# fgnt/pb_chime5

Measured on AMD Instinct MI355X. Metric: utterance-seconds enhanced/sec/GPU (24ch, 20 EM iters), higher is better.
Workload: dtype f64

## Files before the change

### pb_chime5_amd/csrc/gss_api.hip

```cpp
#include <cmath>
#include <cstdarg>
#include <cstdlib>
#include <cstring>
#include <mutex>

#include "gss_internal.h"

#define GSS_ENTER(ctx)                                   \
    if (!(ctx)) return GSS_ERR_INVALID;                  \
    GSS_HIP_CHECK((ctx), hipSetDevice((ctx)->device))
#define GSS_ENTER_VARIANTS(ctx) \
    GSS_ENTER(ctx);             \
    GSS_TRY(variant_refresh(ctx))
static int variant_refresh(gss_ctx *ctx);

#define GSS_STATUS_REF_CHANNEL 0
#define GSS_STATUS_WPE_ZERO_PIVOTS 2

static std::mutex g_error_lock;

int gss_fail(gss_ctx *ctx, int code, const char *fmt, ...) {
    char buf[1024];
    va_list ap;
    va_start(ap, fmt);
    vsnprintf(buf, sizeof(buf), fmt, ap);
    va_end(ap);
    if (ctx) {
        std::lock_guard<std::mutex> guard(g_error_lock);
        ctx->error = buf;
    }
    return code;
}

static thread_local std::string g_create_error;

namespace {
const char *const kVariantKeys[] = {
    "corr_ts", "corr_nw", "corr_blocked", "corr_p_tiles", "chol_diag_unfolded", "apply_ph",
    "apply_generic", "prof_detail", "corr_stg8", "corr_ksplit", "apply_gglobal", "wpe_halves",
    "em_wgs", "estep_wpb", "estep_lds", "mstep_prefetch_d", "mstep_tiled", "mstep_plan_min_d",
    "mstep_chunked", "mstep_slots", "force_eigh", "em_unfused", "em_l3_mb", "em_l3_fit_mb",
    "em_streams", "mstep_maxseg", "em4_cold_eigh", "mstep_generic",
    "wpe_online_mem"};
struct VariantTable {
    std::mutex lock;
    std::string text;
    bool parsed = false;
    std::map<std::string, int> values;
};
VariantTable &variant_table() {
    static VariantTable t;
    return t;
}
}

static int variant_refresh(gss_ctx *ctx) {
    const char *env = getenv("GSS_VARIANT");
    VariantTable &t = variant_table();
    std::lock_guard<std::mutex> guard(t.lock);
    if (t.parsed && t.text == (env ? env : "")) return GSS_OK;
    t.text = env ? env : "";
    t.parsed = true;
// ... 2677 lines not shown
```

### pb_chime5_amd/csrc/wpe.hip

```cpp
#include <algorithm>
#include <cmath>
#include <cstdlib>

#include "gss_internal.h"
#include <type_traits>
#include "dense_wave.h"

typedef double v4d __attribute__((ext_vector_type(4)));

namespace {

constexpr int POW_FRAMES = 256;
__global__ __launch_bounds__(POW_FRAMES) void wpe_power_kernel(const cplx *__restrict__ X,
                                                               int64_t T, int D, int psd_context,
                                                               double *__restrict__ raw,
                                                               double *__restrict__ w) {
    extern __shared__ __attribute__((aligned(16))) char smem[];
    double *ps = reinterpret_cast<double *>(smem);
    __shared__ double red[POW_FRAMES / 64];
    const int f = blockIdx.x, tid = threadIdx.x;
    const cplx *Xf = X + (int64_t)f * T * D;
    double *wout = w + (int64_t)f * T;
    double *wf = psd_context > 0 ? raw + (int64_t)f * T : wout;
    const int DP = D + 1;
// ... 75 lines not shown
                wout[t] = p;
                mx = fmax(mx, p);
            }
        }
    }
    mx = wave_max(mx);
    if ((tid & 63) == 0) red[tid >> 6] = mx;
    __syncthreads();
    mx = fmax(fmax(red[0], red[1]), fmax(red[2], red[3]));
    const double eps = 1e-10 * mx;
    for (int64_t t = tid; t < T; t += POW_FRAMES) wout[t] = 1.0 / fmax(wout[t], eps);
}

#ifndef GSS_CORR_KT
#define GSS_CORR_KT 64
#endif
constexpr int CORR_KT = GSS_CORR_KT;
constexpr int CORR_FINE_MAX_SUBTILES = 48;

struct CorrTile {
    int row_off, col_off, is_p, mask;
};

template <int TS, int MASK, int KSTEPS = CORR_KT / 4>
__device__ __forceinline__ void corr_chunk(const cplx *S, const double *wS, int D,
                                           const CorrTile &tl, v4d (&t1)[TS][TS],
                                           v4d (&t2)[TS][TS], v4d (&t3)[TS][TS]) {
    const int lane = threadIdx.x & 63;
    const int li = lane & 15, lk = lane >> 4;
    auto need = [](int a, int b) { return ((MASK >> (a * TS + b)) & 1) != 0; };
    auto need_row = [&](int a) {
        bool r = false;
        for (int b = 0; b < TS; ++b) r = r || need(a, b);
        return r;
    };
    auto need_col = [&](int b) {
        bool r = false;
        for (int a = 0; a < TS; ++a) r = r || need(a, b);
        return r;
    };
    const int ksteps = KSTEPS;
    cplx a_cur[TS], b_cur[TS], a_nxt[TS], b_nxt[TS];
    double w_cur, w_nxt = 0.0;
    {
        const cplx *base = S + lk * D + li;
        w_cur = wS[lk];
#pragma unroll
        for (int m = 0; m < TS; ++m) {
            a_cur[m] = base[tl.row_off + 16 * m];
            b_cur[m] = base[tl.col_off + 16 * m];
        }
    }
    constexpr int KU = TS == 1 || KSTEPS < 16 ? 4 : 16;
#pragma unroll KU
    for (int ks = 0; ks < ksteps; ++ks) {
        if (ks + 1 < ksteps) {
            const int kf = 4 * (ks + 1) + lk;
            const cplx *base = S + kf * D + li;
            w_nxt = wS[kf];
#pragma unroll
            for (int m = 0; m < TS; ++m) {
                a_nxt[m] = need_row(m) ? base[tl.row_off + 16 * m] : c_make(0.0, 0.0);
                b_nxt[m] = need_col(m) ? base[tl.col_off + 16 * m] : c_make(0.0, 0.0);
            }
        }
        double ar[TS], ai[TS], as[TS], br[TS], bi[TS], bd[TS];
#pragma unroll
        for (int m = 0; m < TS; ++m) {
            ar[m] = a_cur[m].x * w_cur;
            ai[m] = a_cur[m].y * w_cur;
            as[m] = ar[m] + ai[m];
            br[m] = b_cur[m].x;
            bi[m] = b_cur[m].y;
            bd[m] = b_cur[m].x - b_cur[m].y;
        }
#pragma unroll
        for (int a = 0; a < TS; ++a)
#pragma unroll
            for (int b = 0; b < TS; ++b) {
                if (!need(a, b)) continue;
                t1[a][b] = __builtin_amdgcn_mfma_f64_16x16x4f64(ar[a], br[b], t1[a][b], 0, 0, 0);
                t2[a][b] = __builtin_amdgcn_mfma_f64_16x16x4f64(ai[a], bi[b], t2[a][b], 0, 0, 0);
                t3[a][b] = __builtin_amdgcn_mfma_f64_16x16x4f64(as[a], bd[b], t3[a][b], 0, 0, 0);
            }
#pragma unroll
        for (int m = 0; m < TS; ++m) {
            a_cur[m] = a_nxt[m];
            b_cur[m] = b_nxt[m];
        }
        w_cur = w_nxt;
    }
}

template <int TS, int MASK, bool RAW = false>
__device__ __forceinline__ void corr_store(const CorrTile &tl, int f, int n, int c, int D,
                                           const v4d (&t1)[TS][TS], const v4d (&t2)[TS][TS],
                                           const v4d (&t3)[TS][TS], cplx *__restrict__ R,
                                           cplx *__restrict__ P) {
    const int lane = threadIdx.x & 63;
    const int li = lane & 15, lk = lane >> 4;
    auto need = [](int a, int b) { return ((MASK >> (a * TS + b)) & 1) != 0; };
    cplx *Rf = R + (int64_t)f * n * n;
    cplx *Pf = P + (int64_t)f * n * D;
#pragma unroll
    for (int a = 0; a < TS; ++a)
#pragma unroll
        for (int b = 0; b < TS; ++b)
#pragma unroll
            for (int reg = 0; reg < 4; ++reg) {
                if (!need(a, b)) continue;
                const int r = tl.row_off + 16 * a + lk + 4 * reg;
                const int cc = tl.col_off + 16 * b + li;
                const cplx v = RAW ? c_make(t1[a][b][reg], t3[a][b][reg])
                                   : c_make(t1[a][b][reg] + t2[a][b][reg],
                                            (t3[a][b][reg] - t1[a][b][reg]) + t2[a][b][reg]);
                if (r >= n) continue;
                if (tl.is_p == 1) {
                    const int d = cc - c * D;
                    if (d >= 0 && d < D) Pf[r * D + d] = v;
                } else {
                    if (cc < n) Rf[r * n + cc] = v;
                    if (tl.is_p == 2) {
                        const int d = cc - c * D;
                        if (d >= 0 && d < D) Pf[r * D + d] = v;
                    }
                }
            }
}

template <int TS>
__device__ __forceinline__ void corr_zero(v4d (&t1)[TS][TS], v4d (&t2)[TS][TS], v4d (&t3)[TS][TS]) {
#pragma unroll
    for (int a = 0; a < TS; ++a)
#pragma unroll
        for (int b = 0; b < TS; ++b) {
// ... 57 lines not shown
template <int TS, int NW, int STG1 = 8>
__global__ __launch_bounds__(64 * NW, (NW == 1 && STG1 < 8) ? 4 : 1) void wpe_corr_kernel(
    const cplx *__restrict__ Y, const double *__restrict__ w, int F, int64_t T, int D, int n,
    int c, int padf, const CorrTile *__restrict__ tiles, int ntiles, cplx *__restrict__ R,
    cplx *__restrict__ P) {
    extern __shared__ __attribute__((aligned(16))) char smem[];
    const int frames_lds = CORR_KT + c + padf;
    cplx *S = reinterpret_cast<cplx *>(smem);
    double *wS = reinterpret_cast<double *>(S + frames_lds * D);

    int f, grp;
    if (!xcd_group_map((ntiles + NW - 1) / NW, F, f, grp)) return;
    const int wave = __builtin_amdgcn_readfirstlane(threadIdx.x >> 6);
    const int tile_id = grp * NW + wave;
    const bool active = tile_id < ntiles;
    const CorrTile tl = tiles[active ? tile_id : 0];
    const cplx *Yf = Y + (int64_t)f * T * D;
    const double *wf = w + (int64_t)f * T;
    constexpr int FULL = (1 << (TS * TS)) - 1;
    const int mask = __builtin_amdgcn_readfirstlane(active ? tl.mask : 1);
#define CORR_CASE(M) \
    case M: corr_tile_body<TS, M, NW, STG1>(Yf, wf, T, D, n, c, frames_lds, S, wS, tl, active, f, R, P); break
    if (TS == 2) {
        switch (mask) {
            CORR_CASE(1);
            CORR_CASE(3);
            CORR_CASE(5);
            CORR_CASE(11);
            default:
                corr_tile_body<TS, FULL, NW, STG1>(Yf, wf, T, D, n, c, frames_lds, S, wS, tl, active, f, R, P);
        }
    } else {
        corr_tile_body<TS, FULL, NW, STG1>(Yf, wf, T, D, n, c, frames_lds, S, wS, tl, active, f, R, P);
    }
#undef CORR_CASE
}

template <int KS, int STG>
__global__ __launch_bounds__(64 * KS, 4) void wpe_corr_ksplit_kernel(
    const cplx *__restrict__ Y, const double *__restrict__ w, int F, int64_t T, int D, int n,
    int c, int padf, const CorrTile *__restrict__ tiles, int ntiles, cplx *__restrict__ R,
    cplx *__restrict__ P) {
    extern __shared__ __attribute__((aligned(16))) char smem[];
    const int frames_lds = CORR_KT + c + padf;
    const int total = frames_lds * D;
    const size_t wbytes = sizeof(cplx) * (size_t)total + sizeof(double) * CORR_KT;
    int f, tile_id;
// ... 251 lines not shown
        }
    };

    int item = __builtin_amdgcn_readfirstlane(ring[0]);
    if (item < 0) return;
    int b = 0;
    issue(item >> 12, 0, 0);
    __syncthreads();
    for (int k = 0; item >= 0; ++k) {
        const int next = __builtin_amdgcn_readfirstlane(ring[(k + 1) % 3]);
        int fetched = -1;
        if (threadIdx.x == 0 && next >= 0) fetched = corr_fetch(counters, F, xcd, live, cq);
        const int f = item >> 12, grp = item & 4095;
        const int tile_id = grp * NW + wave;
        const bool active = tile_id < ntiles;
        const CorrTile tl = tiles[active ? tile_id : 0];
        const int mask = __builtin_amdgcn_readfirstlane(active ? tl.mask : 1);
        int *ring_slot = &ring[(k + 2) % 3];
#define CORR_CASE(M)                                                                              \
    case M:                                                                                       \
        corr_item_dma<M, NW, BLOCKED>(T, D, n, c, win, S0, w0, tl, active, f, next < 0 ? -1 : next >> 12, \
                                 b, issue, ring_slot, fetched, R, P);                             \
        break
        switch (mask) {
            CORR_CASE(1);
            CORR_CASE(3);
            CORR_CASE(5);
            CORR_CASE(11);
            default:
                corr_item_dma<15, NW, BLOCKED>(T, D, n, c, win, S0, w0, tl, active, f,
                                          next < 0 ? -1 : next >> 12, b, issue, ring_slot, fetched,
                                          R, P);
        }
#undef CORR_CASE
        item = next;
#ifdef GSS_CORR_TRACE
        if (threadIdx.x == 0 && blockIdx.x < 8192) {
            g_corr_trace[blockIdx.x * 6 + 3] = wall_clock64();
            g_corr_trace[blockIdx.x * 6 + 4] = clock64();
            g_corr_trace[blockIdx.x * 6 + 5] = k + 1;
        }
#endif
    }
}

#ifndef GSS_UPD_PREFETCH
#define GSS_UPD_PREFETCH 1
#endif
constexpr int CH_NB = 48;
constexpr int UD_LD = CH_NB + 1;

constexpr size_t DIAG_LDS = sizeof(cplx) * 2 * UD_LD + sizeof(double) * CH_NB;

__device__ inline void chol_diag_block(cplx *A, int n, int j0, cplx *Ud, double *dinv,
                                       int32_t *zero_pivots) {
    const int tid = threadIdx.x, tx = tid & 15, ty = tid >> 4;
    const int nb = min(CH_NB, n - j0);
// ... 439 lines not shown
                    }
                    nxim[it] = -xim[it];
#pragma unroll
                    for (int reg = 0; reg < 4; ++reg) {
                        const int rl = 16 * it + lk + 4 * reg, col = c0 + 16 * b + li;
                        if (rl < nb && col < D)
                            Z[(int64_t)(j0 + rl) * D + col] = c_make(xre[it][reg], xim[it][reg]);
                    }
                }
            }
            __syncthreads();
        }
    }
}

__global__ __launch_bounds__(256, 3) void chol_backsolve_kernel(const cplx *__restrict__ R,
                                                             cplx *__restrict__ P, int n, int D) {
    __shared__ cplx S[CH_NB * BS_LD];
    __shared__ cplx OP[BS_OPS];
    const int f = blockIdx.x;
    chol_backsolve_body(R + (int64_t)f * n * n, P + (int64_t)f * n * D, n, D, S, OP);
}

template <int TA, int NB, int NWV = 4, int WRAPS = 4, bool TAIL = true>
__global__ __launch_bounds__(64 * NWV) void wpe_apply_kernel(const cplx *__restrict__ Y,
                                                        const cplx *__restrict__ G, int F,
                                                        int64_t T, int D, int n, int c,
                                                        cplx *__restrict__ X) {
    constexpr int WAVE_FRAMES = 16 * TA, WG_FRAMES = NWV * WAVE_FRAMES;
    extern __shared__ __attribute__((aligned(16))) char smem[];
    cplx *S = reinterpret_cast<cplx *>(smem);
    const int DP = D | 1;
    int f, chunk;
    if (!xcd_group_map((int)((T + WG_FRAMES - 1) / WG_FRAMES), F, f, chunk)) return;
    const int64_t t0 = (int64_t)chunk * WG_FRAMES;
    const cplx *Yf = Y + (int64_t)f * T * D;
    const cplx *Gf = G + (int64_t)f * n * D;
    const int frames_lds = WG_FRAMES + c + 2;
    const int64_t fr0 = t0 - c;
    constexpr int PRE = 14, NT = 64 * NWV;
    const int total = frames_lds * D;
    for (int base = 0; base < total; base += NT * PRE) {
        cplx v[PRE];
#pragma unroll
        for (int j = 0; j < PRE; ++j) {
            const int idx = base + (int)threadIdx.x + NT * j;
            const int64_t fr = fr0 + idx / D;
            v[j] = c_make(0.0, 0.0);
            if (idx < total && fr >= 0 && fr < T) v[j] = Yf[fr0 * D + idx];
        }
#pragma unroll
        for (int j = 0; j < PRE; ++j) {
            const int idx = base + (int)threadIdx.x + NT * j;
            const int fl = idx / D, d = idx - fl * D;
            if (idx < total) S[fl * DP + d] = v[j];
        }
    }
    __syncthreads();
    const int wave = threadIdx.x >> 6, lane = threadIdx.x & 63;
    const int li = lane & 15, lk = lane >> 4;
    const int wf0 = wave * WAVE_FRAMES;
    if (t0 + wf0 >= T) return;
    v4d acc_re[TA][NB], acc_im[TA][NB], acc_t2[TA][NB];
#pragma unroll
    for (int a = 0; a < TA; ++a)
#pragma unroll
        for (int b = 0; b < NB; ++b) {
            acc_re[a][b] = (v4d){0.0, 0.0, 0.0, 0.0};
            acc_im[a][b] = (v4d){0.0, 0.0, 0.0, 0.0};
            acc_t2[a][b] = (v4d){0.0, 0.0, 0.0, 0.0};
        }
    const int ksteps = (n + 3) / 4;
    const int lds_last = frames_lds * DP - 1;
    int goff[NB], goff_max[NB];
#pragma unroll
    for (int b = 0; b < NB; ++b) {
        const int col = min(16 * b + li, D - 1);
        goff[b] = min(lk, n - 1) * D + col;
        goff_max[b] = (n - 1) * D + col;
    }
    auto load_g = [&](int, cplx (&g)[NB]) {
#pragma unroll
        for (int b = 0; b < NB; ++b) {
            g[b] = Gf[goff[b]];
            goff[b] = min(goff[b] + 4 * D, goff_max[b]);
        }
    };
    int rm = lk % D, lin = (lk / D) * DP + rm;
    int ubase[TA];
#pragma unroll
    for (int a = 0; a < TA; ++a) ubase[a] = (wf0 + 16 * a + li) * DP;
    auto load_u = [&](cplx (&u)[TA]) {
#pragma unroll
        for (int a = 0; a < TA; ++a) u[a] = S[min(ubase[a] + lin, lds_last)];
        rm += 4;
        lin += 4;
#pragma unroll
        for (int w = 0; w < WRAPS; ++w) {
            const bool wrap = rm >= D;
            rm -= wrap ? D : 0;
            lin += wrap ? DP - D : 0;
        }
    };
    auto step = [&](int ks, const cplx (&g)[NB], const cplx (&u)[TA]) {
        const bool ok = !TAIL || 4 * ks + lk < n;
        double ur[TA], ui[TA], gr[NB], gi[NB];
#pragma unroll
        for (int a = 0; a < TA; ++a) {
            ur[a] = ok ? u[a].x : 0.0;
            ui[a] = ok ? u[a].y : 0.0;
        }
#pragma unroll
        for (int b = 0; b < NB; ++b) {
            gr[b] = g[b].x;
            gi[b] = g[b].y;
        }
        double us[TA], gd[NB];
#pragma unroll
        for (int a = 0; a < TA; ++a) us[a] = ur[a] + ui[a];
#pragma unroll
        for (int b = 0; b < NB; ++b) gd[b] = gr[b] - gi[b];
#pragma unroll
        for (int a = 0; a < TA; ++a)
#pragma unroll
            for (int b = 0; b < NB; ++b) {
                acc_re[a][b] = __builtin_amdgcn_mfma_f64_16x16x4f64(ur[a], gr[b], acc_re[a][b], 0, 0, 0);
                acc_t2[a][b] = __builtin_amdgcn_mfma_f64_16x16x4f64(ui[a], gi[b], acc_t2[a][b], 0, 0, 0);
                acc_im[a][b] = __builtin_amdgcn_mfma_f64_16x16x4f64(us[a], gd[b], acc_im[a][b], 0, 0, 0);
            }
    };
    cplx g0[NB], g1[NB], u0[TA], u1[TA];
    load_g(0, g0);
    load_u(u0);
    for (int ks = 0; ks < ksteps; ks += 2) {
        load_g(ks + 1, g1);
        load_u(u1);
        __builtin_amdgcn_sched_barrier(0);
        step(ks, g0, u0);
        __builtin_amdgcn_sched_barrier(0);
        load_g(ks + 2, g0);
        load_u(u0);
        __builtin_amdgcn_sched_barrier(0);
        step(ks + 1, g1, u1);
        __builtin_amdgcn_sched_barrier(0);
    }
#pragma unroll
    for (int a = 0; a < TA; ++a)
#pragma unroll
        for (int b = 0; b < NB; ++b)
#pragma unroll
            for (int reg = 0; reg < 4; ++reg) {
                const int fl = wf0 + 16 * a + lk + 4 * reg;
                const int d = 16 * b + li;
                const int64_t t = t0 + fl;
                if (d < D && t < T) {
                    const cplx y = S[(fl + c) * DP + d];
                    const double pre = acc_re[a][b][reg] + acc_t2[a][b][reg];
                    const double pim = (acc_im[a][b][reg] - acc_re[a][b][reg]) + acc_t2[a][b][reg];
                    X[((int64_t)f * T + t) * D + d] = c_make(y.x - pre, y.y - pim);
                }
            }
}

template <int PH, int NT, bool GLDS = true, int PREW = 14, int PREG = 14>
__global__ __launch_bounds__(256) void wpe_apply_packed_kernel(const cplx *__restrict__ Y,
                                                               const cplx *__restrict__ G, int F,
                                                               int64_t T, int D, int n, int c,
                                                               cplx *__restrict__ X) {
    constexpr int WG_ROWS = 64, WG_FRAMES = PH * WG_ROWS;
    extern __shared__ __attribute__((aligned(16))) char smem[];
    const int DP = D | 1, DG = GLDS ? (D | 1) : D;
    const int frames_lds = WG_FRAMES + c + 2;
    cplx *S = reinterpret_cast<cplx *>(smem);
    cplx *Gl = S + (frames_lds * DP + frames_lds / PH + 1);
    int f, chunk;
    if (!xcd_group_map((int)((T + WG_FRAMES - 1) / WG_FRAMES), F, f, chunk)) return;
    const int64_t t0 = (int64_t)chunk * WG_FRAMES;
    const cplx *Yf = Y + (int64_t)f * T * D;
    const cplx *Gf = G + (int64_t)f * n * D;
    const int64_t fr0 = t0 - c;
    constexpr int NTHR = 256;
    {
        constexpr int PRE = PREW;
        const int total = frames_lds * D;
// ... 195 lines not shown
            const int fl = PH * r + colp[b];
            const int64_t t = t0 + fl;
            if (colv[b] && t < T) {
                const int fw = fl + c;
                const cplx y = S[fw * DP + fw / PH + cold[b]];
                const double pre = acc_re[b][reg] + acc_t2[b][reg];
                const double pim = (acc_im[b][reg] - acc_re[b][reg]) + acc_t2[b][reg];
                X[((int64_t)f * T + t) * D + cold[b]] = c_make(y.x - pre, y.y - pim);
            }
        }
}

__global__ void mfma_selftest_kernel(double *out) {
    const int lane = threadIdx.x;
    const int li = lane & 15, lk = lane >> 4;
    const double a = lk == 0 ? (double)(li + 1) : 0.0;
    const double b = lk == 0 ? 100.0 * (double)(li + 1) : 0.0;
    v4d acc = {0.0, 0.0, 0.0, 0.0};
    acc = __builtin_amdgcn_mfma_f64_16x16x4f64(a, b, acc, 0, 0, 0);
    for (int reg = 0; reg < 4; ++reg) {
        const int row = lk + 4 * reg, col = li;
        out[row * 16 + col] = acc[reg];
    }
}

constexpr int REGROUP_FRAMES = 32;
constexpr int REGROUP_THREADS = 256;

template <bool to_arrays>
__global__ __launch_bounds__(REGROUP_THREADS) void wpe_arrays_regroup_kernel(
    const cplx *__restrict__ src, int64_t T, int A, int C, cplx *__restrict__ dst) {
    __shared__ cplx tile[REGROUP_FRAMES * GSS_MAX_CHANNELS];
    const int D = A * C;
    const int64_t f = blockIdx.y;
    const int64_t t0 = (int64_t)blockIdx.x * REGROUP_FRAMES;
    const int nt = (int)std::min<int64_t>(REGROUP_FRAMES, T - t0);
    const int64_t ftd0 = (f * T + t0) * D;
    const int n_ftd = nt * D;
    if (to_arrays) {
        for (int k = threadIdx.x; k < n_ftd; k += REGROUP_THREADS) tile[k] = src[ftd0 + k];
    } else {
        for (int k = threadIdx.x; k < n_ftd; k += REGROUP_THREADS) {
            const int a = k / (nt * C), r = k - a * nt * C;
            const int t = r / C, c = r - t * C;
            tile[t * D + a * C + c] = src[((f * A + a) * T + t0) * C + r];
        }
// ... 7 lines not shown
        }
    } else {
        for (int k = threadIdx.x; k < n_ftd; k += REGROUP_THREADS) dst[ftd0 + k] = tile[k];
    }
}

}

int wpe_arrays_regroup_run(gss_ctx *ctx, const cplx *src, int F, int64_t T, int A, int C,
                           bool to_arrays, cplx *dst) {
    GSS_REQUIRE(ctx, A * C <= GSS_MAX_CHANNELS, GSS_ERR_UNSUPPORTED, "regroup: D=%d", A * C);
    const dim3 grid((unsigned)((T + REGROUP_FRAMES - 1) / REGROUP_FRAMES), (unsigned)F);
    GSS_PROF(ctx, "wpe_arrays_regroup");
    if (to_arrays)
        hipLaunchKernelGGL(wpe_arrays_regroup_kernel<true>, grid, dim3(REGROUP_THREADS), 0,
                           ctx->stream, src, T, A, C, dst);
    else
        hipLaunchKernelGGL(wpe_arrays_regroup_kernel<false>, grid, dim3(REGROUP_THREADS), 0,
                           ctx->stream, src, T, A, C, dst);
    GSS_LAUNCH_CHECK(ctx, "wpe_arrays_regroup_kernel");
    return GSS_OK;
}

static int corr_tiles(int n, int D, int c, int ct, std::vector<CorrTile> &tiles) {
    const int ts = ct / 16;
    auto mask_of = [&](int r0, int c0, int ncols_limit, bool upper_only) {
        int m = 0;
        for (int a = 0; a < ts; ++a)
            for (int b = 0; b < ts; ++b) {
                const int rr = r0 + 16 * a, cc = c0 + 16 * b;
                bool needed = rr < n && cc < ncols_limit;
                if (upper_only && cc + 15 < rr) needed = false;
                if (needed) m |= 1 << (a * ts + b);
            }
        return m;
    };
    const int last_col = (n - 1) / ct;
    const bool p_folded = ct == 16 && (c * D) / ct == last_col && (c * D + D - 1) / ct == last_col &&
                          !gss_variant_set("corr_p_tiles");
    for (int r0 = 0; r0 < n; r0 += ct)
        for (int c0 = 0; c0 < n; c0 += ct)
            if (c0 + ct > r0) {
                const bool with_p = p_folded && c0 / ct == last_col;
                tiles.push_back({r0, c0, with_p ? 2 : 0,
                                 mask_of(r0, c0, with_p ? std::max(n, c * D + D) : n, true)});
            }
    if (!p_folded)
        for (int r0 = 0; r0 < n; r0 += ct)
            for (int c0 = 0; c0 < D; c0 += ct)
                tiles.push_back({r0, c * D + c0, 1, mask_of(r0, c0, D, false)});
    std::stable_sort(tiles.begin(), tiles.end(), [](const CorrTile &x, const CorrTile &y) {
        return __builtin_popcount(x.mask) > __builtin_popcount(y.mask);
    });
    return (int)tiles.size();
}

static int corr_tiles_pairs(int n, int D, int c, std::vector<CorrTile> &tiles) {
    for (int r0 = 0; r0 < n; r0 += 16)
        for (int c0 = r0; c0 < n; c0 += 32) tiles.push_back({r0, c0, 0, c0 + 16 < n ? 3 : 1});
    for (int r0 = 0; r0 < n; r0 += 32)
        for (int c0 = 0; c0 < D; c0 += 16) tiles.push_back({r0, c * D + c0, 1, r0 + 16 < n ? 5 : 1});
    std::stable_sort(tiles.begin(), tiles.end(), [](const CorrTile &x, const CorrTile &y) {
        return __builtin_popcount(x.mask) > __builtin_popcount(y.mask);
    });
    return (int)tiles.size();
}

static int corr_padf(int D, int ct) { return (ct + D - 1) / D + 1; }

struct WpeWork {
    double *w, *raw;
    cplx *R, *P;
};
static WpeWork wpe_blocks(Workspace &ws, int F, int64_t T, int D, int taps, bool own_w,
                          bool smoothed) {
// ... 51 lines not shown
        if (X != Y)
            GSS_HIP_CHECK(ctx, hipMemcpyAsync(X, Y, sizeof(cplx) * (size_t)F * T * D,
                                              hipMemcpyDeviceToDevice, ctx->stream));
        return GSS_OK;
    }
    GSS_REQUIRE(ctx, X != Y, GSS_ERR_INVALID, "gss_wpe: X must not alias Y");
    GSS_REQUIRE(ctx, !cw || (cw->w && iterations == 1 && part < 0), GSS_ERR_INVALID,
                "wpe: the caller's weights serve one iteration of a whole call");
    Workspace ws(ctx);
    const WpeWork k = wpe_blocks(ws, F, T, D, taps, !cw, psd_context > 0);
    GSS_TRY(ws.status("wpe"));
    double *w_own = k.w, *raw = k.raw;
    const double *w = cw ? cw->w : w_own;
    cplx *R = k.R, *P = k.P;

    std::vector<CorrTile> tiles;
    const int sub16 = (n + 15) / 16;
    int corr_ts = sub16 * (sub16 + 1) / 2 + sub16 * ((D + 15) / 16) <= CORR_FINE_MAX_SUBTILES ? 1 : 2;
    bool corr_pairs = false;
    if (const int e = gss_variant("corr_ts", 0)) {
        corr_ts = e == 1 ? 1 : 2;
        corr_pairs = e == 3;
    }
    const int ntiles = corr_pairs ? corr_tiles_pairs(n, D, c, tiles) : corr_tiles(n, D, c, 16 * corr_ts, tiles);
    constexpr int tm16 = 16, tn16 = 16;
    std::vector<UpdTile> upd;
    std::vector<int> upd_start, upd_count, upd_j0, upd_k, upd_ndiag;
    const bool fold_diag = !gss_variant_set("chol_diag_unfolded");
    {
        const int nblk = (n + CH_NB - 1) / CH_NB;
        for (int J = 0; J < nblk; ++J) {
            upd_start.push_back((int)upd.size());
            const int rs = (J + 1) * CH_NB;
            const bool narrow = J % 2 == 0;
            const int r_end = narrow ? std::min(rs + CH_NB, n) : n;
            const int d_end = std::min(rs + CH_NB, n);
            for (int r0 = rs; r0 < d_end; r0 += tm16)
                for (int c0 = rs; c0 < d_end; c0 += tn16)
                    if (c0 + tn16 > r0) upd.push_back({r0, c0, 0, 0});
            upd_ndiag.push_back(fold_diag ? (int)upd.size() - upd_start.back() : 0);
            for (int r0 = rs; r0 < r_end; r0 += tm16) {
                for (int c0 = rs; c0 < n; c0 += tn16)
                    if (c0 + tn16 > r0 && !(r0 < d_end && c0 < d_end)) upd.push_back({r0, c0, 0, 0});
                for (int cc = 0; cc < D; cc += tn16) upd.push_back({r0, cc, 1, 0});
            }
            upd_count.push_back((int)upd.size() - upd_start.back());
            const bool wide = J % 2 == 1;
            upd_j0.push_back(wide ? (J - 1) * CH_NB : J * CH_NB);
            upd_k.push_back(wide ? 2 * CH_NB : CH_NB);
        }
    }
    GSS_REQUIRE(ctx, ntiles <= 1024 && upd.size() <= 4096, GSS_ERR_UNSUPPORTED,
                "wpe: taps*D=%d too large", n);
    static_assert(sizeof(CorrTile) == sizeof(UpdTile), "tile structs share one buffer");
    if (ctx->wpe_tiles_key[0] != taps || ctx->wpe_tiles_key[1] != delay ||
        ctx->wpe_tiles_key[2] != D || ctx->wpe_tiles_key[3] != corr_ts + (fold_diag ? 0 : 16) + (corr_pairs ? 32 : 0)) {
        GSS_HIP_CHECK(ctx, hipStreamSynchronize(ctx->stream));
        if (!ctx->wpe_tiles)
            GSS_HIP_CHECK(ctx, hipMalloc(&ctx->wpe_tiles, sizeof(CorrTile) * (1024 + 4096 + 1 + 64)));
        if (ctx->debug_pattern >= 0)
            GSS_HIP_CHECK(ctx, hipMemset(ctx->wpe_tiles, ctx->debug_pattern,
                                         sizeof(CorrTile) * (1024 + 4096 + 1 + 64)));
        GSS_HIP_CHECK(ctx, hipMemcpy(ctx->wpe_tiles, tiles.data(), sizeof(CorrTile) * ntiles,
                                     hipMemcpyHostToDevice));
        if (!upd.empty())
            GSS_HIP_CHECK(ctx, hipMemcpy(reinterpret_cast<CorrTile *>(ctx->wpe_tiles) + 1024,
                                         upd.data(), sizeof(UpdTile) * upd.size(),
                                         hipMemcpyHostToDevice));
        ctx->wpe_tiles_key[0] = taps;
        ctx->wpe_tiles_key[1] = delay;
        ctx->wpe_tiles_key[2] = D;
        ctx->wpe_tiles_key[3] = corr_ts + (fold_diag ? 0 : 16) + (corr_pairs ? 32 : 0);
    }
    CorrTile *tiles_dev = reinterpret_cast<CorrTile *>(ctx->wpe_tiles);
    UpdTile *upd_dev = reinterpret_cast<UpdTile *>(tiles_dev + 1024);
    int32_t *zero_pivots = reinterpret_cast<int32_t *>(tiles_dev + 1024 + 4096);
    if (part <= 0 && !(cw && cw->accumulate))
        GSS_HIP_CHECK(ctx, hipMemsetAsync(zero_pivots, 0, sizeof(int32_t), ctx->stream));
    if (part == 0) GSS_HIP_CHECK(ctx, hipEventRecord(ctx->ev_fork, ctx->stream));
    int *corr_counters = reinterpret_cast<int *>(tiles_dev + 1024 + 4096 + 1) + (part == 1 ? 128 : 0);

    const int padf = corr_padf(D, 16 * corr_ts);
    const size_t corr_lds_probe = sizeof(cplx) * (size_t)(CORR_KT + c + corr_padf(D, 16 * corr_ts)) * D +
                                  sizeof(double) * CORR_KT;
    auto round_eff = [&](int nw) {
        const double wgs = (double)((ntiles + nw - 1) / nw) * F;
        const int by_regs = 16 / nw, by_lds = (int)(160 * 1024 / corr_lds_probe);
        const double rounds = wgs / (256.0 * std::max(1, std::min(by_regs, by_lds)));
        return rounds / std::ceil(rounds);
    };
    int corr_nw = corr_ts == 2 && round_eff(2) > round_eff(4) + 0.15 ? 2 : 4;
    const int nw_forced = gss_variant("corr_nw", 0);
    if (nw_forced) corr_nw = nw_forced == 2 ? 2 : nw_forced == 1 && corr_ts == 1 ? 1 : 4;
    if (corr_ts == 1 && (size_t)(CORR_KT + c + padf) * D <= 512 && !nw_forced) corr_nw = 1;
    const bool corr_stg5 = (size_t)(CORR_KT + c + padf) * D <= 320 && !gss_variant_set("corr_stg8");
// ... 9 lines not shown
    const bool corr_split = ksplit_forced ? ksplit_forced != 1 : !arrays_single_waves;
    const int corr_ks = (corr_ts == 1 && corr_nw == 1 && corr_split)
                            ? (ksplit_forced == 2 ? 2 : 4) : 1;
    using corr_fn_t = void (*)(const cplx *, const double *, int, int64_t, int, int, int, int,
                               const CorrTile *, int, cplx *, cplx *);
    corr_fn_t ksplit_fn = nullptr;
    if (corr_ks > 1) {
        ksplit_fn = corr_stg5 ? (corr_ks == 2 ? wpe_corr_ksplit_kernel<2, 5> : wpe_corr_ksplit_kernel<4, 5>)
                              : (corr_ks == 2 ? wpe_corr_ksplit_kernel<2, 8> : wpe_corr_ksplit_kernel<4, 8>);
        corr_lds = std::max(corr_lds * corr_ks, sizeof(cplx) * 256 * (size_t)(corr_ks - 1));
    }
    const size_t panel_lds = sizeof(cplx) * UDP_SIZE + sizeof(double) * CH_NB;
    constexpr int apply_ta = 2;
    constexpr int apply_nwv = 4;
    const int apply_frames = 16 * apply_ta * apply_nwv;
    auto apply_fn = D <= 16 ? wpe_apply_kernel<apply_ta, 1> : wpe_apply_kernel<apply_ta, 2>;
    if (D >= 4 && !gss_variant_set("apply_generic")) {
        if (n % 8 == 0)
            apply_fn = D <= 16 ? wpe_apply_kernel<apply_ta, 1, 4, 1, false>
                               : wpe_apply_kernel<apply_ta, 2, 4, 1, false>;
        else
            apply_fn = D <= 16 ? wpe_apply_kernel<apply_ta, 1, 4, 1, true>
                               : wpe_apply_kernel<apply_ta, 2, 4, 1, true>;
    }
    const size_t apply_lds = sizeof(cplx) * (size_t)(apply_frames + c + 2) * (D | 1);
    int apply_ph = 1, apply_nt = (D + 15) / 16;
    size_t packed_lds = 0;
    {
        const int ph_env = gss_variant("apply_ph", 0);
        bool ph_env_taken = ph_env <= 1;
        double best = (double)((D + 15) / 16) * n;
        for (int ph = 2; ph <= 4; ++ph) {
            if (ph_env > 0 && ph != ph_env) continue;
            const int nt = (ph * D + 15) / 16;
            if (nt > 3 || D < 2) continue;
            const double cost = (double)nt * (n + (ph - 1) * D) / ph;
            const int fl = 64 * ph + c + 2;
            const size_t lds = sizeof(cplx) * ((size_t)fl * (D | 1) + fl / ph + 1 + (size_t)(n + 1) * (D | 1));
            if (lds > (ph_env == ph ? 160 : 64) * 1024) continue;
            if (cost < 0.75 * best || ph_env == ph) {
                ph_env_taken = ph_env_taken || ph_env == ph;
                best = cost;
                apply_ph = ph;
                apply_nt = nt;
                packed_lds = lds;
            }
// ... 40 lines not shown
                "wpe: taps=%d D=%d needs more LDS than a CU has", taps, D);
    if (apply_lds > 64 * 1024)
        GSS_HIP_CHECK(ctx, hipFuncSetAttribute(reinterpret_cast<const void *>(apply_fn),
                                               hipFuncAttributeMaxDynamicSharedMemorySize,
                                               (int)apply_lds));
    if (corr_lds > 64 * 1024)
        GSS_HIP_CHECK(ctx, hipFuncSetAttribute(reinterpret_cast<const void *>(corr_fn),
                                               hipFuncAttributeMaxDynamicSharedMemorySize,
                                               (int)corr_lds));
    const int corr_pieces = (int)(((size_t)(CORR_KT + c + padf) * D + 63) / 64);
    const size_t corr_dma_lds = 2 * (sizeof(cplx) * 64 * (size_t)corr_pieces + sizeof(double) * CORR_KT);
    const bool corr_persist = corr_ts == 2 && (int64_t)T * D * 16 < (1LL << 31) &&
                              corr_dma_lds <= 80 * 1024;
    if (corr_persist && !nw_forced) corr_nw = 4;
    const bool corr_blocked = corr_persist && gss_variant_set("corr_blocked");
    auto corr_persist_fn = corr_blocked ? (corr_nw == 2 ? wpe_corr_persist_kernel<2, true>
                                                        : wpe_corr_persist_kernel<4, true>)
                                        : (corr_nw == 2 ? wpe_corr_persist_kernel<2>
                                                        : wpe_corr_persist_kernel<4>);
    CorrQueue corr_queue{(ntiles + corr_nw - 1) / corr_nw, 0};
    int corr_slots = 0;
    if (corr_persist) {
        for (int g = 0; g < corr_queue.ngroups; ++g)
            if (__builtin_popcount(tiles[g * corr_nw].mask) >= 3) corr_queue.gh = g + 1;
        if (corr_dma_lds > 64 * 1024)
            GSS_HIP_CHECK(ctx, hipFuncSetAttribute(reinterpret_cast<const void *>(corr_persist_fn),
                                                   hipFuncAttributeMaxDynamicSharedMemorySize,
                                                   (int)corr_dma_lds));
        int per_cu = 0, cus = 0;
        GSS_HIP_CHECK(ctx, hipOccupancyMaxActiveBlocksPerMultiprocessor(
                               &per_cu, reinterpret_cast<const void *>(corr_persist_fn), 64 * corr_nw,
                               corr_dma_lds));
        GSS_HIP_CHECK(ctx, hipDeviceGetAttribute(&cus, hipDeviceAttributeMultiprocessorCount, ctx->device));
        corr_slots = std::min(std::max(per_cu, 1) * cus, corr_queue.ngroups * F);
    }

    for (int it = 0; it < iterations; ++it) {
        const cplx *cur = it == 0 ? Y : X;
        if (!cw) {
            GSS_PROF(ctx, "wpe_power");
            GSS_TRY(wpe_power_launch(ctx, cur, F, T, D, psd_context, raw, w_own));
        }
        if (corr_persist) {
            GSS_HIP_CHECK(ctx, hipMemsetAsync(corr_counters, 0, 8 * 16 * sizeof(int), ctx->stream));
            GSS_PROF(ctx, "wpe_corr");
            hipLaunchKernelGGL(corr_persist_fn, dim3(corr_slots), dim3(64 * corr_nw), corr_dma_lds,
                               ctx->stream, Y, w, F, T, D, n, c, corr_pieces, tiles_dev, ntiles,
// ... 64 lines not shown
                                   dim3(64 * apply_nwv), apply_lds, ctx->stream, Y, P, F, T, D, n, c, X);
            }
            GSS_LAUNCH_CHECK(ctx, "wpe_apply_kernel");
        }
    }
    if (part < 0)
        GSS_HIP_CHECK(ctx, hipMemcpyAsync(ctx->status_host + (cw ? cw->status_word : 2), zero_pivots,
                                          sizeof(int32_t), hipMemcpyDeviceToHost, ctx->stream));
    return GSS_OK;
}


int wpe_copy_zero_pivots(gss_ctx *ctx) {
    if (!ctx->wpe_tiles) return GSS_OK;
    const int32_t *zero_pivots =
        reinterpret_cast<const int32_t *>(reinterpret_cast<const CorrTile *>(ctx->wpe_tiles) + 1024 + 4096);
    GSS_HIP_CHECK(ctx, hipMemcpyAsync(ctx->status_host + 2, zero_pivots, sizeof(int32_t),
                                      hipMemcpyDeviceToHost, ctx->stream));
    return GSS_OK;
}

int selftest_mfma_run(gss_ctx *ctx) {
    double *out = nullptr;
    GSS_HIP_CHECK(ctx, hipMalloc(reinterpret_cast<void **>(&out), sizeof(double) * 256));
    hipLaunchKernelGGL(mfma_selftest_kernel, dim3(1), dim3(64), 0, ctx->stream, out);
    double host[256];
    hipError_t e = hipMemcpyAsync(host, out, sizeof(host), hipMemcpyDeviceToHost, ctx->stream);
    if (e == hipSuccess) e = hipStreamSynchronize(ctx->stream);
    (void)hipFree(out);
    if (e != hipSuccess) return gss_fail(ctx, GSS_ERR_HIP, "mfma selftest: %s", hipGetErrorString(e));
    for (int i = 0; i < 16; ++i)
        for (int j = 0; j < 16; ++j) {
            const double want = (double)(i + 1) * 100.0 * (double)(j + 1);
            if (host[i * 16 + j] != want)
                return gss_fail(ctx, GSS_ERR_UNSUPPORTED,
                                "f64 MFMA fragment layout mismatch at (%d,%d): got %g want %g", i,
                                j, host[i * 16 + j], want);
        }
    return GSS_OK;
}
```

### pb_chime5_amd/roofline.py

```python

PEAK_HBM_GBS = 8000.0
PEAK_F64_TFLOPS = 78.6
MEASURED_F64_MFMA_TFLOPS = 77.6
MEASURED_WPE_CORR_MIX_TFLOPS = 73.5
PEAK_SMEM_BYTES_PER_CYCLE_PER_CU = 3.27
NUM_CUS = 256
NUM_SIMDS = 1024
CLOCK_GHZ = 2.4
VALU_F64_ISSUE_CYCLES = 4.0


def estep_scalar_bytes(F, T, D, K):
    return 16.0 * (D * (D + 1) // 2) * K * F * -(-T // 64)


def estep_valu_instructions(F, T, D, K):
    return (D * (D + 1) // 2) * (4.0 + 2.0 * K) * F * -(-T // 64)


def stft_bin_bytes(F, T, D):
    return 16.0 * F * T * D


def kernel_work(name, *, F, T, D, K, taps, N, iterations=20):
    BY = stft_bin_bytes(F, T, D)
    n = taps * D
    if name == 'wpe_corr':
        need = n * (n + 1) // 2 + n * D
        sub = -(-n // 16)
        subtiles = sub * (sub + 1) // 2 + sub * -(-D // 16)
        c = (n // D) + 1 if D else 0
        if D <= 12 and (c * D) // 16 == (c * D + D - 1) // 16 == sub - 1:
            subtiles = sub * (sub + 1) // 2
        rem = T % 64
        t_exec = T - rem + (0 if rem == 0 else 64 if rem > 48 or subtiles <= 48
                            else 16 * -(-rem // 16))
        return dict(flops=F * 6.0 * need * T, bytes=BY + 8.0 * F * T + 16.0 * F * need,
                    bound='mfma',
                    dense_flops=F * (8.0 * n * n * T + 8.0 * n * D * T),
                    executed_flops=F * 6.0 * subtiles * 256 * t_exec)
    if name == 'wpe_solve':
        return dict(flops=F * ((8.0 / 3.0) * n ** 3 + 8.0 * n * n * D),
                    bytes=16.0 * F * (n * n + 2 * n * D), bound='mfma')
    if name == 'wpe_apply':
        return dict(flops=F * 8.0 * D * n * T, bytes=2 * BY + 16.0 * F * n * D, bound='mfma')
    if name == 'wpe_power':
        return dict(flops=F * T * 3.0 * D, bytes=BY + 8.0 * F * T, bound='hbm')
    if name in ('em_estep', 'em_predict', 'em_mstep'):
        NE = D * (D + 1) // 2
        dense = (4.0 if name == 'em_mstep' else 8.0) * D * D * K * F * T
        return dict(flops=F * T * NE * (6.0 + 4.0 * K), bytes=BY + 8.0 * F * K * T,
                    bound='valu_f64', dense_flops=dense)
    if name == 'em_onchip':
        NE = D * (D + 1) // 2
        passes = iterations + 1
        return dict(flops=passes * 2 * F * T * NE * (6.0 + 4.0 * K), bytes=passes * BY,
# ... 96 lines not shown
```

Measured before the change: 1086.

## Use 4x4x4 f64 MFMA remainder groups for partial channel tiles in WPE

When the channel count D is between 17 and 28, the second 16-wide column tile in the WPE correlation P-tiles and in the apply kernel is only partly used. That tile is replaced by one to three 4x4x4 f64 MFMA groups that cover just the remaining channels, so less wasted MFMA work is issued. Tile cost ordering and the persistent-queue heavy-group threshold are updated to match. The mfma self-test gains a 4x4x4 fragment layout check. The change adds kernel template variants and more complex indexing, and it can be turned off with the remainder_full_tile variant flag.

```diff
diff --git a/pb_chime5_amd/csrc/gss_api.hip b/pb_chime5_amd/csrc/gss_api.hip
--- a/pb_chime5_amd/csrc/gss_api.hip
+++ b/pb_chime5_amd/csrc/gss_api.hip
@@ -38,6 +38,7 @@
 const char *const kVariantKeys[] = {
     "corr_ts", "corr_nw", "corr_blocked", "corr_p_tiles", "chol_diag_unfolded", "apply_ph",
     "apply_generic", "prof_detail", "corr_stg8", "corr_ksplit", "apply_gglobal", "wpe_halves",
+    "remainder_full_tile",
     "em_wgs", "estep_wpb", "estep_lds", "mstep_prefetch_d", "mstep_tiled", "mstep_plan_min_d",
     "mstep_chunked", "mstep_slots", "force_eigh", "em_unfused", "em_l3_mb", "em_l3_fit_mb",
     "em_streams", "mstep_maxseg", "em4_cold_eigh", "mstep_generic",
diff --git a/pb_chime5_amd/csrc/wpe.hip b/pb_chime5_amd/csrc/wpe.hip
--- a/pb_chime5_amd/csrc/wpe.hip
+++ b/pb_chime5_amd/csrc/wpe.hip
@@ -121,12 +121,15 @@
     int row_off, col_off, is_p, mask;
 };
 
+constexpr int corr_rg(int TS, int MASK) { return TS == 2 ? (MASK >> 4) & 3 : 0; }
+
 template <int TS, int MASK, int KSTEPS = CORR_KT / 4>
 __device__ __forceinline__ void corr_chunk(const cplx *S, const double *wS, int D,
                                            const CorrTile &tl, v4d (&t1)[TS][TS],
                                            v4d (&t2)[TS][TS], v4d (&t3)[TS][TS]) {
     const int lane = threadIdx.x & 63;
     const int li = lane & 15, lk = lane >> 4;
+    constexpr int RG = corr_rg(TS, MASK), NG = RG > 0 ? RG : 1;
     auto need = [](int a, int b) { return ((MASK >> (a * TS + b)) & 1) != 0; };
     auto need_row = [&](int a) {
         bool r = false;
@@ -136,18 +139,24 @@
     auto need_col = [&](int b) {
         bool r = false;
         for (int a = 0; a < TS; ++a) r = r || need(a, b);
-        return r;
+        return r && !(RG > 0 && b == 1);
     };
     const int ksteps = KSTEPS;
     cplx a_cur[TS], b_cur[TS], a_nxt[TS], b_nxt[TS];
+    cplx g_cur[NG], g_nxt[NG];
     double w_cur, w_nxt = 0.0;
+    const int goff = tl.col_off + 16 + (lane & 3);
     {
         const cplx *base = S + lk * D + li;
         w_cur = wS[lk];
 #pragma unroll
         for (int m = 0; m < TS; ++m) {
             a_cur[m] = base[tl.row_off + 16 * m];
-            b_cur[m] = base[tl.col_off + 16 * m];
+            b_cur[m] = need_col(m) || RG == 0 ? base[tl.col_off + 16 * m] : c_make(0.0, 0.0);
+        }
+        if constexpr (RG > 0) {
+#pragma unroll
+            for (int g = 0; g < RG; ++g) g_cur[g] = S[lk * D + goff + 4 * g];
         }
     }
     constexpr int KU = TS == 1 || KSTEPS < 16 ? 4 : 16;
@@ -162,6 +171,10 @@
                 a_nxt[m] = need_row(m) ? base[tl.row_off + 16 * m] : c_make(0.0, 0.0);
                 b_nxt[m] = need_col(m) ? base[tl.col_off + 16 * m] : c_make(0.0, 0.0);
             }
+            if constexpr (RG > 0) {
+#pragma unroll
+                for (int g = 0; g < RG; ++g) g_nxt[g] = S[kf * D + goff + 4 * g];
+            }
         }
         double ar[TS], ai[TS], as[TS], br[TS], bi[TS], bd[TS];
 #pragma unroll
@@ -178,6 +191,18 @@
 #pragma unroll
             for (int b = 0; b < TS; ++b) {
                 if (!need(a, b)) continue;
+                if constexpr (RG > 0) {
+                    if (b == 1) {
+#pragma unroll
+                        for (int g = 0; g < RG; ++g) {
+                            const double gr = g_cur[g].x, gi = g_cur[g].y;
+                            t1[a][1][g] = __builtin_amdgcn_mfma_f64_4x4x4f64(ar[a], gr, t1[a][1][g], 0, 0, 0);
+                            t2[a][1][g] = __builtin_amdgcn_mfma_f64_4x4x4f64(ai[a], gi, t2[a][1][g], 0, 0, 0);
+                            t3[a][1][g] = __builtin_amdgcn_mfma_f64_4x4x4f64(as[a], gr - gi, t3[a][1][g], 0, 0, 0);
+                        }
+                        continue;
+                    }
+                }
                 t1[a][b] = __builtin_amdgcn_mfma_f64_16x16x4f64(ar[a], br[b], t1[a][b], 0, 0, 0);
                 t2[a][b] = __builtin_amdgcn_mfma_f64_16x16x4f64(ai[a], bi[b], t2[a][b], 0, 0, 0);
                 t3[a][b] = __builtin_amdgcn_mfma_f64_16x16x4f64(as[a], bd[b], t3[a][b], 0, 0, 0);
@@ -186,6 +211,10 @@
         for (int m = 0; m < TS; ++m) {
             a_cur[m] = a_nxt[m];
             b_cur[m] = b_nxt[m];
+        }
+        if constexpr (RG > 0) {
+#pragma unroll
+            for (int g = 0; g < RG; ++g) g_cur[g] = g_nxt[g];
         }
         w_cur = w_nxt;
     }
@@ -208,8 +237,11 @@
 #pragma unroll
             for (int reg = 0; reg < 4; ++reg) {
                 if (!need(a, b)) continue;
-                const int r = tl.row_off + 16 * a + lk + 4 * reg;
-                const int cc = tl.col_off + 16 * b + li;
+                constexpr int RG = corr_rg(TS, MASK);
+                const bool small = RG > 0 && b == 1;
+                if (small && reg >= RG) continue;
+                const int r = tl.row_off + 16 * a + (small ? 4 * ((lane >> 2) & 3) + lk : lk + 4 * reg);
+                const int cc = tl.col_off + 16 * b + (small ? 4 * reg + (lane & 3) : li);
                 const cplx v = RAW ? c_make(t1[a][b][reg], t3[a][b][reg])
                                    : c_make(t1[a][b][reg] + t2[a][b][reg],
                                             (t3[a][b][reg] - t1[a][b][reg]) + t2[a][b][reg]);
@@ -313,7 +345,7 @@
 #define CORR_CASE(M) \
     case M: corr_tile_body<TS, M, NW, STG1>(Yf, wf, T, D, n, c, frames_lds, S, wS, tl, active, f, R, P); break
     if (TS == 2) {
-        switch (mask) {
+        switch (mask & 15) {
             CORR_CASE(1);
             CORR_CASE(3);
             CORR_CASE(5);
@@ -611,17 +643,28 @@
         corr_item_dma<M, NW, BLOCKED>(T, D, n, c, win, S0, w0, tl, active, f, next < 0 ? -1 : next >> 12, \
                                  b, issue, ring_slot, fetched, R, P);                             \
         break
-        switch (mask) {
+#define CORR_CASE_RG(RG)                                                                          \
+    case 15 + 16 * RG:                                                                            \
+        if constexpr (!BLOCKED)                                                                   \
+            corr_item_dma<15 + 16 * RG, NW, false>(T, D, n, c, win, S0, w0, tl, active, f,        \
+                                                   next < 0 ? -1 : next >> 12, b, issue,          \
+                                                   ring_slot, fetched, R, P);                     \
+        break
+        switch (BLOCKED ? mask & 15 : mask) {
             CORR_CASE(1);
             CORR_CASE(3);
             CORR_CASE(5);
             CORR_CASE(11);
+            CORR_CASE_RG(1);
+            CORR_CASE_RG(2);
+            CORR_CASE_RG(3);
             default:
                 corr_item_dma<15, NW, BLOCKED>(T, D, n, c, win, S0, w0, tl, active, f,
                                           next < 0 ? -1 : next >> 12, b, issue, ring_slot, fetched,
                                           R, P);
         }
 #undef CORR_CASE
+#undef CORR_CASE_RG
         item = next;
 #ifdef GSS_CORR_TRACE
         if (threadIdx.x == 0 && blockIdx.x < 8192) {
@@ -1107,11 +1150,10 @@
     chol_backsolve_body(R + (int64_t)f * n * n, P + (int64_t)f * n * D, n, D, S, OP);
 }
 
-template <int TA, int NB, int NWV = 4, int WRAPS = 4, bool TAIL = true>
-__global__ __launch_bounds__(64 * NWV) void wpe_apply_kernel(const cplx *__restrict__ Y,
-                                                        const cplx *__restrict__ G, int F,
-                                                        int64_t T, int D, int n, int c,
-                                                        cplx *__restrict__ X) {
+template <int TA, int NB, int NWV, int WRAPS, bool TAIL, int RG>
+__device__ __forceinline__ void wpe_apply_body(const cplx *__restrict__ Y,
+                                               const cplx *__restrict__ G, int F, int64_t T, int D,
+                                               int n, int c, cplx *__restrict__ X) {
     constexpr int WAVE_FRAMES = 16 * TA, WG_FRAMES = NWV * WAVE_FRAMES;
     extern __shared__ __attribute__((aligned(16))) char smem[];
     cplx *S = reinterpret_cast<cplx *>(smem);
@@ -1146,27 +1188,35 @@
     const int li = lane & 15, lk = lane >> 4;
     const int wf0 = wave * WAVE_FRAMES;
     if (t0 + wf0 >= T) return;
-    v4d acc_re[TA][NB], acc_im[TA][NB], acc_t2[TA][NB];
-#pragma unroll
-    for (int a = 0; a < TA; ++a)
-#pragma unroll
-        for (int b = 0; b < NB; ++b) {
+    static_assert(RG == 0 || NB == 2, "remainder groups replace the second of two channel tiles");
+    constexpr int NBL = RG > 0 ? 1 : NB;
+    constexpr int NG = RG > 0 ? RG : 1;
+    v4d acc_re[TA][NBL], acc_im[TA][NBL], acc_t2[TA][NBL];
+    double sml_re[TA][NG], sml_im[TA][NG], sml_t2[TA][NG];
+#pragma unroll
+    for (int a = 0; a < TA; ++a) {
+#pragma unroll
+        for (int b = 0; b < NBL; ++b) {
             acc_re[a][b] = (v4d){0.0, 0.0, 0.0, 0.0};
             acc_im[a][b] = (v4d){0.0, 0.0, 0.0, 0.0};
             acc_t2[a][b] = (v4d){0.0, 0.0, 0.0, 0.0};
         }
+#pragma unroll
+        for (int g = 0; g < NG; ++g) sml_re[a][g] = sml_im[a][g] = sml_t2[a][g] = 0.0;
+    }
     const int ksteps = (n + 3) / 4;
     const int lds_last = frames_lds * DP - 1;
-    int goff[NB], goff_max[NB];
-#pragma unroll
-    for (int b = 0; b < NB; ++b) {
-        const int col = min(16 * b + li, D - 1);
+    constexpr int NBG = NBL + RG;
+    int goff[NBG], goff_max[NBG];
+#pragma unroll
+    for (int b = 0; b < NBG; ++b) {
+        const int col = min(b < NBL ? 16 * b + li : 16 + 4 * (b - NBL) + (lane & 3), D - 1);
         goff[b] = min(lk, n - 1) * D + col;
         goff_max[b] = (n - 1) * D + col;
     }
-    auto load_g = [&](int, cplx (&g)[NB]) {
-#pragma unroll
-        for (int b = 0; b < NB; ++b) {
+    auto load_g = [&](int, cplx (&g)[NBG]) {
+#pragma unroll
+        for (int b = 0; b < NBG; ++b) {
             g[b] = Gf[goff[b]];
             goff[b] = min(goff[b] + 4 * D, goff_max[b]);
         }
@@ -1187,34 +1237,42 @@
             lin += wrap ? DP - D : 0;
         }
     };
-    auto step = [&](int ks, const cplx (&g)[NB], const cplx (&u)[TA]) {
+    auto step = [&](int ks, const cplx (&g)[NBG], const cplx (&u)[TA]) {
         const bool ok = !TAIL || 4 * ks + lk < n;
-        double ur[TA], ui[TA], gr[NB], gi[NB];
+        double ur[TA], ui[TA], gr[NBG], gi[NBG];
 #pragma unroll
         for (int a = 0; a < TA; ++a) {
             ur[a] = ok ? u[a].x : 0.0;
             ui[a] = ok ? u[a].y : 0.0;
         }
 #pragma unroll
-        for (int b = 0; b < NB; ++b) {
+        for (int b = 0; b < NBG; ++b) {
             gr[b] = g[b].x;
             gi[b] = g[b].y;
         }
-        double us[TA], gd[NB];
+        double us[TA], gd[NBG];
 #pragma unroll
         for (int a = 0; a < TA; ++a) us[a] = ur[a] + ui[a];
 #pragma unroll
-        for (int b = 0; b < NB; ++b) gd[b] = gr[b] - gi[b];
-#pragma unroll
-        for (int a = 0; a < TA; ++a)
-#pragma unroll
-            for (int b = 0; b < NB; ++b) {
+        for (int b = 0; b < NBG; ++b) gd[b] = gr[b] - gi[b];
+#pragma unroll
+        for (int a = 0; a < TA; ++a) {
+#pragma unroll
+            for (int b = 0; b < NBL; ++b) {
                 acc_re[a][b] = __builtin_amdgcn_mfma_f64_16x16x4f64(ur[a], gr[b], acc_re[a][b], 0, 0, 0);
                 acc_t2[a][b] = __builtin_amdgcn_mfma_f64_16x16x4f64(ui[a], gi[b], acc_t2[a][b], 0, 0, 0);
                 acc_im[a][b] = __builtin_amdgcn_mfma_f64_16x16x4f64(us[a], gd[b], acc_im[a][b], 0, 0, 0);
             }
+#pragma unroll
+            for (int g = 0; g < RG; ++g) {
+                const int b = NBL + g;
+                sml_re[a][g] = __builtin_amdgcn_mfma_f64_4x4x4f64(ur[a], gr[b], sml_re[a][g], 0, 0, 0);
+                sml_t2[a][g] = __builtin_amdgcn_mfma_f64_4x4x4f64(ui[a], gi[b], sml_t2[a][g], 0, 0, 0);
+                sml_im[a][g] = __builtin_amdgcn_mfma_f64_4x4x4f64(us[a], gd[b], sml_im[a][g], 0, 0, 0);
+            }
+        }
     };
-    cplx g0[NB], g1[NB], u0[TA], u1[TA];
+    cplx g0[NBG], g1[NBG], u0[TA], u1[TA];
     load_g(0, g0);
     load_u(u0);
     for (int ks = 0; ks < ksteps; ks += 2) {
@@ -1232,7 +1290,7 @@
 #pragma unroll
     for (int a = 0; a < TA; ++a)
 #pragma unroll
-        for (int b = 0; b < NB; ++b)
+        for (int b = 0; b < NBL; ++b)
 #pragma unroll
             for (int reg = 0; reg < 4; ++reg) {
                 const int fl = wf0 + 16 * a + lk + 4 * reg;
@@ -1245,6 +1303,36 @@
                     X[((int64_t)f * T + t) * D + d] = c_make(y.x - pre, y.y - pim);
                 }
             }
+#pragma unroll
+    for (int a = 0; a < TA; ++a)
+#pragma unroll
+        for (int g = 0; g < RG; ++g) {
+            const int fl = wf0 + 16 * a + 4 * ((lane >> 2) & 3) + (lane >> 4);
+            const int d = 16 + 4 * g + (lane & 3);
+            const int64_t t = t0 + fl;
+            if (d < D && t < T) {
+                const cplx y = S[(fl + c) * DP + d];
+                const double pre = sml_re[a][g] + sml_t2[a][g];
+                const double pim = (sml_im[a][g] - sml_re[a][g]) + sml_t2[a][g];
+                X[((int64_t)f * T + t) * D + d] = c_make(y.x - pre, y.y - pim);
+            }
+        }
+}
+
+template <int TA, int NB, int NWV = 4, int WRAPS = 4, bool TAIL = true>
+__global__ __launch_bounds__(64 * NWV) void wpe_apply_kernel(const cplx *__restrict__ Y,
+                                                        const cplx *__restrict__ G, int F,
+                                                        int64_t T, int D, int n, int c,
+                                                        cplx *__restrict__ X) {
+    wpe_apply_body<TA, NB, NWV, WRAPS, TAIL, 0>(Y, G, F, T, D, n, c, X);
+}
+
+template <int TA, int RG, bool TAIL>
+__global__ __launch_bounds__(256) void wpe_apply_rg_kernel(const cplx *__restrict__ Y,
+                                                           const cplx *__restrict__ G, int F,
+                                                           int64_t T, int D, int n, int c,
+                                                           cplx *__restrict__ X) {
+    wpe_apply_body<TA, 2, 4, 1, TAIL, RG>(Y, G, F, T, D, n, c, X);
 }
 
 template <int PH, int NT, bool GLDS = true, int PREW = 14, int PREG = 14>
@@ -1486,6 +1574,9 @@
         const int row = lk + 4 * reg, col = li;
         out[row * 16 + col] = acc[reg];
     }
+    double d = 0.0;
+    d = __builtin_amdgcn_mfma_f64_4x4x4f64((double)(lane + 1), 100.0 * (double)(lane + 1), d, 0, 0, 0);
+    out[256 + lane] = d;
 }
 
 constexpr int REGROUP_FRAMES = 32;
@@ -1539,7 +1630,13 @@
     return GSS_OK;
 }
 
-static int corr_tiles(int n, int D, int c, int ct, std::vector<CorrTile> &tiles) {
+static int corr_tile_cost(const CorrTile &t) {
+    const int rg = (t.mask >> 4) & 3;
+    if (rg == 0) return 4 * __builtin_popcount(t.mask & 15);
+    return 4 * __builtin_popcount(t.mask & 5) + rg * __builtin_popcount(t.mask & 10);
+}
+
+static int corr_tiles(int n, int D, int c, int ct, bool small_p, std::vector<CorrTile> &tiles) {
     const int ts = ct / 16;
     auto mask_of = [&](int r0, int c0, int ncols_limit, bool upper_only) {
         int m = 0;
@@ -1564,10 +1661,13 @@
             }
     if (!p_folded)
         for (int r0 = 0; r0 < n; r0 += ct)
-            for (int c0 = 0; c0 < D; c0 += ct)
-                tiles.push_back({r0, c * D + c0, 1, mask_of(r0, c0, D, false)});
+            for (int c0 = 0; c0 < D; c0 += ct) {
+                int m = mask_of(r0, c0, D, false);
+                if (small_p && ct == 32 && m == 15 && D > 16 && D <= 28) m |= ((D - 16 + 3) / 4) << 4;
+                tiles.push_back({r0, c * D + c0, 1, m});
+            }
     std::stable_sort(tiles.begin(), tiles.end(), [](const CorrTile &x, const CorrTile &y) {
-        return __builtin_popcount(x.mask) > __builtin_popcount(y.mask);
+        return corr_tile_cost(x) > corr_tile_cost(y);
     });
     return (int)tiles.size();
 }
@@ -1665,7 +1765,9 @@
         corr_ts = e == 1 ? 1 : 2;
         corr_pairs = e == 3;
     }
-    const int ntiles = corr_pairs ? corr_tiles_pairs(n, D, c, tiles) : corr_tiles(n, D, c, 16 * corr_ts, tiles);
+    const bool remainder_full_tile = gss_variant_set("remainder_full_tile");
+    const int ntiles = corr_pairs ? corr_tiles_pairs(n, D, c, tiles)
+                                  : corr_tiles(n, D, c, 16 * corr_ts, !remainder_full_tile, tiles);
     constexpr int tm16 = 16, tn16 = 16;
     std::vector<UpdTile> upd;
     std::vector<int> upd_start, upd_count, upd_j0, upd_k, upd_ndiag;
@@ -1697,7 +1799,7 @@
                 "wpe: taps*D=%d too large", n);
     static_assert(sizeof(CorrTile) == sizeof(UpdTile), "tile structs share one buffer");
     if (ctx->wpe_tiles_key[0] != taps || ctx->wpe_tiles_key[1] != delay ||
-        ctx->wpe_tiles_key[2] != D || ctx->wpe_tiles_key[3] != corr_ts + (fold_diag ? 0 : 16) + (corr_pairs ? 32 : 0)) {
+        ctx->wpe_tiles_key[2] != D || ctx->wpe_tiles_key[3] != corr_ts + (fold_diag ? 0 : 16) + (corr_pairs ? 32 : 0) + (remainder_full_tile ? 64 : 0)) {
         GSS_HIP_CHECK(ctx, hipStreamSynchronize(ctx->stream));
         if (!ctx->wpe_tiles)
             GSS_HIP_CHECK(ctx, hipMalloc(&ctx->wpe_tiles, sizeof(CorrTile) * (1024 + 4096 + 1 + 64)));
@@ -1713,7 +1815,7 @@
         ctx->wpe_tiles_key[0] = taps;
         ctx->wpe_tiles_key[1] = delay;
         ctx->wpe_tiles_key[2] = D;
-        ctx->wpe_tiles_key[3] = corr_ts + (fold_diag ? 0 : 16) + (corr_pairs ? 32 : 0);
+        ctx->wpe_tiles_key[3] = corr_ts + (fold_diag ? 0 : 16) + (corr_pairs ? 32 : 0) + (remainder_full_tile ? 64 : 0);
     }
     CorrTile *tiles_dev = reinterpret_cast<CorrTile *>(ctx->wpe_tiles);
     UpdTile *upd_dev = reinterpret_cast<UpdTile *>(tiles_dev + 1024);
@@ -1769,6 +1871,14 @@
         else
             apply_fn = D <= 16 ? wpe_apply_kernel<apply_ta, 1, 4, 1, true>
                                : wpe_apply_kernel<apply_ta, 2, 4, 1, true>;
+        using apply_t = decltype(apply_fn);
+        static const apply_t table_rg[2][3] = {
+            {wpe_apply_rg_kernel<apply_ta, 1, false>, wpe_apply_rg_kernel<apply_ta, 2, false>,
+             wpe_apply_rg_kernel<apply_ta, 3, false>},
+            {wpe_apply_rg_kernel<apply_ta, 1, true>, wpe_apply_rg_kernel<apply_ta, 2, true>,
+             wpe_apply_rg_kernel<apply_ta, 3, true>}};
+        if (D > 16 && D <= 28 && !remainder_full_tile)
+            apply_fn = table_rg[n % 8 == 0 ? 0 : 1][(D - 16 + 3) / 4 - 1];
     }
     const size_t apply_lds = sizeof(cplx) * (size_t)(apply_frames + c + 2) * (D | 1);
     int apply_ph = 1, apply_nt = (D + 15) / 16;
@@ -1855,7 +1965,7 @@
     int corr_slots = 0;
     if (corr_persist) {
         for (int g = 0; g < corr_queue.ngroups; ++g)
-            if (__builtin_popcount(tiles[g * corr_nw].mask) >= 3) corr_queue.gh = g + 1;
+            if (corr_tile_cost(tiles[g * corr_nw]) >= 12) corr_queue.gh = g + 1;
         if (corr_dma_lds > 64 * 1024)
             GSS_HIP_CHECK(ctx, hipFuncSetAttribute(reinterpret_cast<const void *>(corr_persist_fn),
                                                    hipFuncAttributeMaxDynamicSharedMemorySize,
@@ -1966,9 +2076,9 @@
 
 int selftest_mfma_run(gss_ctx *ctx) {
     double *out = nullptr;
-    GSS_HIP_CHECK(ctx, hipMalloc(reinterpret_cast<void **>(&out), sizeof(double) * 256));
+    GSS_HIP_CHECK(ctx, hipMalloc(reinterpret_cast<void **>(&out), sizeof(double) * 320));
     hipLaunchKernelGGL(mfma_selftest_kernel, dim3(1), dim3(64), 0, ctx->stream, out);
-    double host[256];
+    double host[320];
     hipError_t e = hipMemcpyAsync(host, out, sizeof(host), hipMemcpyDeviceToHost, ctx->stream);
     if (e == hipSuccess) e = hipStreamSynchronize(ctx->stream);
     (void)hipFree(out);
@@ -1981,5 +2091,17 @@
                                 "f64 MFMA fragment layout mismatch at (%d,%d): got %g want %g", i,
                                 j, host[i * 16 + j], want);
         }
+    for (int q = 0; q < 4; ++q)
+        for (int i = 0; i < 4; ++i)
+            for (int j = 0; j < 4; ++j) {
+                double want = 0.0;
+                for (int k = 0; k < 4; ++k)
+                    want += (double)(1 + i + 4 * q + 16 * k) * 100.0 * (double)(1 + j + 4 * q + 16 * k);
+                const double got = host[256 + j + 4 * q + 16 * i];
+                if (got != want)
+                    return gss_fail(ctx, GSS_ERR_UNSUPPORTED,
+                                    "f64 4x4x4 MFMA fragment layout mismatch at block %d (%d,%d): got %g want %g",
+                                    q, i, j, got, want);
+            }
     return GSS_OK;
 }
diff --git a/pb_chime5_amd/roofline.py b/pb_chime5_amd/roofline.py
--- a/pb_chime5_amd/roofline.py
+++ b/pb_chime5_amd/roofline.py
@@ -32,6 +32,9 @@
         c = (n // D) + 1 if D else 0
         if D <= 12 and (c * D) // 16 == (c * D + D - 1) // 16 == sub - 1:
             subtiles = sub * (sub + 1) // 2
+        if 16 < D <= 28 and subtiles > 48:
+            whole = max(0, -(-(n - 16) // 32))
+            subtiles -= 2 * whole * (1 - -(-(D - 16) // 4) / 4.0)
         rem = T % 64
         t_exec = T - rem + (0 if rem == 0 else 64 if rem > 48 or subtiles <= 48
                             else 16 * -(-rem // 16))
```

Result: faster. 1111, median of 6 (+2.3%).
